# hallgeirl/cse168-raytracer

Measured on AMD Instinct MI355X. Metric: Mrays/s (primary+shadow), higher is better.
Workload: dtype f32; 1 GPU; sponza-standin 1920x1080 64spp primary+shadow; scene_triangles=76552, bvh_nodes=46701, math=exact: every quotient of the reference's slab and triangle tests, bit for bit, control_flow=while-while, ray_order=image order, resident_bytes_per_gpu=35765164

## Files before the change

cse168-raytracer_amd/csrc/mr_frame.hip:

```cpp
#include <hip/hip_runtime.h>

#include <cstring>

#include "mr_eye.h"
#include "mr_internal.h"
#include "mr_launch.h"
#include "mr_phong.h"
#include "mr_recursion.h"
#include "mr_surface.h"
#include "mr_tile.h"
#include "mr_traverse.h"

namespace mr {
namespace {

struct FrameArgs {
    EyeFrame eye;
    TraceParams tp;
    SurfacePtrs m;
    DirectLight lt;
    const float *mats;
    const uint32_t *prim_mat;
    mr_hit *hits;
    mr_hit *shadow_hits;
// ... 6 lines not shown
    uint32_t build, n_inner, n_rec;
};

__device__ __forceinline__ void eye_tables(const FrameArgs &a) {
    const unsigned i = blockIdx.x * (unsigned)kTraceBlock + threadIdx.x;
    const float ex = a.eye.eye[0], ey = a.eye.eye[1], ez = a.eye.eye[2];
    if (i < a.n_inner) {
        const float4 *q = a.tp.nodes + 4 * (size_t)i;
        const float4 q0 = q[0], q1 = q[1], q2 = q[2];
        int4 q3 = *reinterpret_cast<const int4 *>(q + 3);
        if (!(regular_pos(ex) && regular_pos(ey) && regular_pos(ez))) q3.z |= 1;
        float4 *d = a.rel_nodes + 4 * (size_t)i;
        d[0] = make_float4(q0.x - ex, q0.y - ex, q0.z - ey, q0.w - ey);
        d[1] = make_float4(q1.x - ex, q1.y - ex, q1.z - ey, q1.w - ey);
        d[2] = make_float4(q2.x - ez, q2.y - ez, q2.z - ez, q2.w - ez);
        *reinterpret_cast<int4 *>(d + 3) = q3;
    }
    if (i < a.n_rec) {
        const float4 *q = a.tp.tris + 3 * (size_t)i;
        const float4 q0 = q[0], q1 = q[1], q2 = q[2];
        const TriOriginTerms o = tri_origin_terms(q0, q1, q2, ex, ey, ez);
        float4 *d = a.rel_tris + 3 * (size_t)i;
        d[0] = make_float4(q2.y, q2.z, q2.w, o.pn);
        d[1] = make_float4(o.u.x, o.u.y, o.u.z, o.w.x);
        d[2] = make_float4(o.w.y, o.w.z, 0.0f, 0.0f);
    }
}

__device__ __forceinline__ unsigned tail_first_run(unsigned body_iters) {
    const unsigned q = body_iters >> 2;
    return q >= 8u ? 8u : q >= 4u ? 4u : q >= 2u ? 2u : 1u;
}
template <typename T>
__device__ __forceinline__ T kernarg_now(size_t offset) {
    typedef const volatile T __attribute__((address_space(4))) *ptr_t;
    const char __attribute__((address_space(4))) *ka = (const char __attribute__((address_space(4))) *)__builtin_amdgcn_kernarg_segment_ptr();
    return *(ptr_t)(ka + offset);
}

#ifndef MIRO_TAIL_PERMILLE
#define MIRO_TAIL_PERMILLE 60
#endif
#ifndef MIRO_BODY_ITERS
#define MIRO_BODY_ITERS 32
#endif
#ifndef MIRO_TAIL_MIN_CHUNKS
#define MIRO_TAIL_MIN_CHUNKS 60000ull
#endif
constexpr uint32_t kTailWgs = 1792 * (256 / kTraceBlock);
#ifndef MIRO_BODY_MIN_WGS
#define MIRO_BODY_MIN_WGS 14000
#endif
#ifndef MIRO_TAIL_PERMILLE_MID
#define MIRO_TAIL_PERMILLE_MID 60
#define MIRO_BODY_MIN_WGS_MID 14000
#endif
constexpr uint32_t kBodyMinWgs = MIRO_BODY_MIN_WGS;
struct FrameShape { uint32_t body_wgs, body_iters, tail_chunks, grid; };
inline FrameShape frame_schedule(unsigned long long chunks) {
    FrameShape s;
    if (chunks < MIRO_TAIL_MIN_CHUNKS || MIRO_TAIL_PERMILLE == 0 || kTraceBlock != 256) {
        const unsigned long long cap = chunks < kFrameLargeChunks ? (unsigned long long)kTraceGridCap : (unsigned long long)kFrameGridCapLarge;
        s.body_wgs = (uint32_t)(chunks < cap ? chunks : cap);
        s.body_iters = (uint32_t)((chunks + s.body_wgs - 1) / s.body_wgs);
        s.tail_chunks = 0;
        s.grid = s.body_wgs;
        return s;
    }
    const bool mid = chunks < kFrameLargeChunks;
    const unsigned long long tail_target = chunks * (mid ? MIRO_TAIL_PERMILLE_MID : MIRO_TAIL_PERMILLE) / 1000;
    uint32_t m = MIRO_BODY_ITERS;
    while (m > 1 && (chunks - tail_target) / m < (mid ? (uint32_t)MIRO_BODY_MIN_WGS_MID : kBodyMinWgs)) m >>= 1;
    while ((unsigned long long)m * (unsigned long long)kFrameGridCapLarge < chunks) m <<= 1;
    s.body_iters = m;
    s.body_wgs = (uint32_t)((chunks - tail_target) / m);
    s.tail_chunks = (uint32_t)(chunks - (unsigned long long)s.body_wgs * m);
    s.grid = s.body_wgs + kTailWgs;
    return s;
}

#if defined(MIRO_WG_TIMES) && MIRO_TRACE_BLOCK == 256
__device__ unsigned long long g_wg_times[4 * 131072];
#endif
template <int VAR, int SHADOW, bool MAT>
#ifndef MIRO_FRAME_WAVES
#define MIRO_FRAME_WAVES 7
#endif
__global__ __launch_bounds__(kTraceBlock) __attribute__((amdgpu_waves_per_eu(MIRO_FRAME_WAVES, 8))) void frame_kernel(FrameArgs a) {
#if defined(MIRO_WG_TIMES) && MIRO_TRACE_BLOCK == 256
    const unsigned long long wg_t0 = wall_clock64();
#endif
    constexpr bool kEyeRel = VAR == kTraceEyeRel;
    if (kEyeRel && a.build) {
        eye_tables(a);
        return;
    }
    extern __shared__ int s_stack[];
    __shared__ unsigned s_shadow_rays[kTraceBlock / 64];
    const int tid = threadIdx.x;
    const unsigned long long n = a.eye.n, n_round = (n + 63ull) & ~63ull;
    constexpr bool kObj = (VAR & kVarObjects) != 0;
    const uint32_t spp = a.eye.spp;
    const float inv_spp = 1.0f / (float)spp;
    Stats st = {0ull, 0ull};
    unsigned my_shadow_rays = 0;

    __shared__ unsigned s_pull, s_run[2];
    if (tid == 0) { s_run[0] = 0; s_run[1] = 0; }
    unsigned long long idx, stride, limit;
    if (blockIdx.x < a.body_wgs) {
        const unsigned long long body_end = (unsigned long long)a.body_wgs * a.body_iters * kTraceBlock;
        idx = (unsigned long long)xcd_block_id_of(blockIdx.x, a.body_wgs, a.body_wgs >= (unsigned)kFrameGridCapLarge || a.tail_chunks != 0, a.tail_chunks != 0 ? 4096u : kXcdMinGrid) * kTraceBlock + tid;
        stride = (unsigned long long)a.body_wgs * kTraceBlock;
        limit = body_end < n_round ? body_end : n_round;
    } else {
        idx = 0; stride = 0; limit = n_round;
    }
    for (;; idx += stride) {
        if (__builtin_expect(stride == 0, 0)) {
            if (tid == 0) {
                unsigned left = s_run[1], next = s_run[0] + 1u;
                if (left == 0) {
                    const unsigned T = kernarg_now<uint32_t>(offsetof(FrameArgs, tail_chunks));
                    unsigned k = atomicAdd(kernarg_now<unsigned *>(offsetof(FrameArgs, tail_counter)), 1u);
                    s_pull = k;
                    unsigned at = 0;
                    next = 0xFFFFFFFFu;
                    for (unsigned size = tail_first_run(kernarg_now<uint32_t>(offsetof(FrameArgs, body_iters))); size >= 1; size >>= 1) {
                        const unsigned runs = size > 1 ? T / (4u * size) : T - at;
                        if (k < runs) { next = at + k * size; left = size; break; }
                        k -= runs;
                        at += runs * size;
                    }
                }
                s_run[0] = next;
                s_run[1] = next == 0xFFFFFFFFu ? 0u : left - 1u;
            }
            __syncthreads();
            const unsigned c = s_run[0];
            __syncthreads();
            if (c == 0xFFFFFFFFu) break;
            idx = ((unsigned long long)kernarg_now<uint32_t>(offsetof(FrameArgs, tail_base)) + c) * kTraceBlock + tid;
            if (idx >= limit) continue;
        } else if (idx >= limit) break;
        const bool live = idx < n;
        uint32_t x = 0, row = 0, y = 0, sm = 0;
        float4 ra = make_float4(0.f, 0.f, 0.f, 0.f), rb = make_float4(1.f, 1.f, 1.f, -1.f);
        if (live) {
            eye_sample_of(a.eye, idx, x, row, y, sm);
            eye_ray_of(a.eye, x, y, sm, ra, rb);
        }
        mr_hit h;
        {
            RayRegs r;
            ray_setup(r, ra, rb);
            Lane L;
            int plane_hit;
            if (kEyeRel) {
                TraceParams tp = a.tp;
                tp.nodes = a.rel_nodes; tp.tris = a.rel_tris;
                for (int k = 0; k < 3; k++) {
                    tp.root_lo[k] = kernarg_now<float>(offsetof(FrameArgs, rel_root_lo) + 4 * k);
                    tp.root_hi[k] = kernarg_now<float>(offsetof(FrameArgs, rel_root_hi) + 4 * k);
                }
                trace_ray<true, false, false, VAR, kEyeRel>(tp, r, rb.w, live, L, plane_hit, s_stack, tid, st);
            } else {
                trace_ray<true, false, false, VAR>(a.tp, r, rb.w, live, L, plane_hit, s_stack, tid, st);
            }
            h = make_hit<kObj>(a.tp, L, plane_hit, rb.w);
        }
        if (a.hits && live) reinterpret_cast<float4 *>(a.hits)[idx] = *reinterpret_cast<const float4 *>(&h);

        const bool hit = live && h.prim != MR_MISS;
        float c[3] = {0.f, 0.f, 0.f}, highlight = 0.0f;
        if (live && !hit) { c[0] = a.lt.bg[0]; c[1] = a.lt.bg[1]; c[2] = a.lt.bg[2]; }
        float4 sa = make_float4(0.f, 0.f, 0.f, 0.f), sb = make_float4(1.f, 1.f, 1.f, -1.f);
        if (hit) {
            float P[3], N[3];
            const float ox = kEyeRel ? a.eye.eye[0] : ra.x, oy = kEyeRel ? a.eye.eye[1] : ra.y, oz = kEyeRel ? a.eye.eye[2] : ra.z;
            if (MAT) {
                rec::MeshMat mm;
                mm.s = a.m; mm.mats = a.mats; mm.prim_mat = a.prim_mat;
                LightArgs la;
                for (int k = 0; k < 3; k++) { la.L[k] = a.lt.L[k]; la.color[k] = a.lt.color[k]; }
                la.wattage = a.lt.wattage;
                rec::surface_point_od(mm, ox, oy, oz, rb.x, rb.y, rb.z, h.t, h.prim, h.beta, h.gamma, P, N);
                phong_terms(la, rec::material_of(mm, h.prim), P, N, rb.x, rb.y, rb.z, c, highlight);
            } else {
                surface_od<true>(a.m, ox, oy, oz, rb.x, rb.y, rb.z, h.t, h.prim, h.beta, h.gamma, P, N);
            }
            if (SHADOW != 2) shadow_ray_of(P, a.lt.L[0], a.lt.L[1], a.lt.L[2], sa, sb);
            if (!MAT) phong_direct(a.lt, P, N, rb.x, rb.y, rb.z, c);
            if (SHADOW != 2) my_shadow_rays++;
        }
        if (SHADOW != 2) {
            RayRegs r;
            ray_setup(r, sa, sb);
            Lane L;
            int plane_hit;
            trace_ray<true, SHADOW == 1, false, VAR>(a.tp, r, sb.w, hit, L, plane_hit, s_stack, tid, st);
            mr_hit hs = make_hit<kObj>(a.tp, L, plane_hit, sb.w);
            if (!hit) { hs.t = 0.0f; hs.prim = MR_MISS; hs.beta = 0.0f; hs.gamma = 0.0f; }
            if (a.shadow_hits && live) reinterpret_cast<float4 *>(a.shadow_hits)[idx] = *reinterpret_cast<const float4 *>(&hs);
            if (MAT) {
                if (hit) {
                    rec::MeshMat mm;
                    mm.s = a.m; mm.mats = a.mats; mm.prim_mat = a.prim_mat;
                    phong_combine(c, highlight, light_scale_of(mm, sa, sb, *reinterpret_cast<const float4 *>(&hs)), c);
                }
            } else if (hs.prim != MR_MISS) {
                c[0] = 0.f; c[1] = 0.f; c[2] = 0.f;
            }
        } else {
            if (a.shadow_hits && live) reinterpret_cast<float4 *>(a.shadow_hits)[idx] = make_float4(0.0f, __uint_as_float(MR_MISS), 0.0f, 0.0f);
            if (MAT && hit) phong_combine(c, highlight, 1.0f, c);
        }
        for (uint32_t off = 1; off < spp; off <<= 1) {
            c[0] += __shfl_xor(c[0], (int)off, 64);
            c[1] += __shfl_xor(c[1], (int)off, 64);
            c[2] += __shfl_xor(c[2], (int)off, 64);
        }
        if (live) eye_sample_of(a.eye, idx, x, row, y, sm);
        if (live && sm == 0) {
            if (spp > 1) { c[0] *= inv_spp; c[1] *= inv_spp; c[2] *= inv_spp; }
            float *o = a.rgb + 3 * ((size_t)row * a.eye.W + x);
            o[0] = c[0]; o[1] = c[1]; o[2] = c[2];
        }
    }

    if (stride == 0 && tid == 0) {
        const unsigned readers = gridDim.x - kernarg_now<uint32_t>(offsetof(FrameArgs, body_wgs));
        const unsigned T = kernarg_now<uint32_t>(offsetof(FrameArgs, tail_chunks));
        unsigned runs = 0, at = 0;
        for (unsigned size = tail_first_run(kernarg_now<uint32_t>(offsetof(FrameArgs, body_iters))); size >= 1; size >>= 1) {
            const unsigned r = size > 1 ? T / (4u * size) : T - at;
            runs += r;
            at += r * size;
        }
        if (s_pull == runs + readers - 1u) atomicExch(kernarg_now<unsigned *>(offsetof(FrameArgs, tail_counter)), 0u);
    }
    if (a.counts) {
        unsigned w = my_shadow_rays;
        for (int off = 32; off > 0; off >>= 1) w += __shfl_down(w, off, 64);
        if ((tid & 63) == 0) s_shadow_rays[tid >> 6] = w;
        __syncthreads();
        if (tid == 0) {
            unsigned long long tot = 0;
            for (int k = 0; k < kTraceBlock / 64; k++) tot += s_shadow_rays[k];
            if (tot) atomicAdd(&a.counts[1], tot);
            if (blockIdx.x == 0) atomicAdd(&a.counts[0], n);
        }
    }
#if defined(MIRO_WG_TIMES) && MIRO_TRACE_BLOCK == 256
    if (tid == 0 && blockIdx.x < 131072u) {
        g_wg_times[4 * blockIdx.x] = wg_t0;
        g_wg_times[4 * blockIdx.x + 1] = wall_clock64();
        g_wg_times[4 * blockIdx.x + 2] = __builtin_amdgcn_s_getreg((31 << 11) | 4);
        g_wg_times[4 * blockIdx.x + 3] = __builtin_amdgcn_s_getreg((31 << 11) | 20);
    }
#endif
}
#if defined(MIRO_WG_TIMES) && MIRO_TRACE_BLOCK == 256
}
}
extern "C" int mr_debug_wg_times(unsigned long long *out, unsigned n_words) {
    return (int)hipMemcpyFromSymbol(out, HIP_SYMBOL(mr::g_wg_times), (size_t)n_words * 8, 0, hipMemcpyDeviceToHost);
}
namespace mr {
namespace {
#endif

template <int VAR, int SHADOW, bool MAT>
mr_status launch_frame_t(FrameArgs a, hipStream_t stream) {
    size_t lds = 0;
    const mr_status st = stack_lds(&frame_kernel<VAR, SHADOW, MAT>, a.tp.stack_depth, kStackLdsShared, lds);
    if (st != MR_OK) return st;
    const FrameShape shape = frame_schedule((a.eye.n + kTraceBlock - 1) / kTraceBlock);
    a.body_wgs = shape.body_wgs; a.body_iters = shape.body_iters; a.tail_chunks = shape.tail_chunks;
    a.tail_base = shape.body_wgs * shape.body_iters;
    if (shape.tail_chunks && !a.tail_counter) return fail(MR_ERR_STATE, "mr_render_direct: no hand-out counter for the tail of a large frame");
    hipLaunchKernelGGL((frame_kernel<VAR, SHADOW, MAT>), dim3(shape.grid), dim3(kTraceBlock), lds, stream, a);
    MR_HIP_CHECK(hipGetLastError());
    return MR_OK;
}

template <int VAR>
mr_status launch_frame_plain(const FrameArgs &a, bool any, hipStream_t stream) {
    return any ? launch_frame_t<VAR, 1, false>(a, stream) : launch_frame_t<VAR, 0, false>(a, stream);
}
template <int VAR>
mr_status launch_frame_default(const FrameArgs &a, bool any, bool no_shadows, bool mat, hipStream_t stream) {
    if (mat) return no_shadows ? launch_frame_t<VAR, 2, true>(a, stream) : launch_frame_t<VAR, 0, true>(a, stream);
    if (no_shadows) return launch_frame_t<VAR, 2, false>(a, stream);
    return launch_frame_plain<VAR>(a, any, stream);
}

}

#ifndef MR_FRAME_ENTRY
#define MR_FRAME_ENTRY launch_frame_b256
#endif
static mr_status eye_tables_for(const DeviceScene &ds, EyeTablePool &pool, FrameArgs &a, hipStream_t stream) {
    hipStreamCaptureStatus cs = hipStreamCaptureStatusNone;
    MR_HIP_CHECK(hipStreamIsCapturing(stream, &cs));
    const bool capturing = cs != hipStreamCaptureStatusNone;
    std::lock_guard<std::mutex> lock(pool.mu);
    const uint64_t call = ++pool.calls;
    EyeTables *e = nullptr;
    if (!capturing)
        for (EyeTables &c : pool.set)
            if (c.reusable && memcmp(c.eye, a.eye.eye, sizeof(c.eye)) == 0) { e = &c; break; }
    const bool build = e == nullptr;
    if (build) {
        e = &pool.set[0];
        for (EyeTables &c : pool.set)
            if (c.last_use < e->last_use) e = &c;
        e->reusable = false;
        if (!e->d || !e->ready) {
            hipStreamCaptureMode mode = hipStreamCaptureModeRelaxed;
            MR_HIP_CHECK(hipThreadExchangeStreamCaptureMode(&mode));
            hipError_t err = e->d ? hipSuccess : hipMalloc(reinterpret_cast<void **>(&e->d), eye_table_bytes(ds));
            if (err == hipSuccess && !e->ready)
                err = hipEventCreateWithFlags(reinterpret_cast<hipEvent_t *>(&e->ready), hipEventDisableTiming);
            MR_HIP_CHECK(hipThreadExchangeStreamCaptureMode(&mode));
            MR_HIP_CHECK(err);
        }
    } else if (e->stream != (void *)stream) {
        MR_HIP_CHECK(hipStreamWaitEvent(stream, static_cast<hipEvent_t>(e->ready), 0));
    }
    e->last_use = call;
    a.rel_nodes = e->d;
    a.rel_tris = e->d + 4 * (size_t)ds.n_inner;
    for (int c = 0; c < 3; c++) { a.rel_root_lo[c] = ds.root_lo[c] - a.eye.eye[c]; a.rel_root_hi[c] = ds.root_hi[c] - a.eye.eye[c]; }
    if (!build) return MR_OK;
    FrameArgs b = a;
    b.build = 1; b.n_inner = ds.n_inner; b.n_rec = ds.n_tris;
    const uint32_t n = ds.n_inner > ds.n_tris ? ds.n_inner : ds.n_tris;
    if (n) {
        hipLaunchKernelGGL((frame_kernel<kTraceEyeRel, 0, false>), dim3((n + kTraceBlock - 1) / kTraceBlock), dim3(kTraceBlock), 0, stream, b);
        MR_HIP_CHECK(hipGetLastError());
    }
    if (capturing) e->captured = true;
    if (!e->captured) {
        MR_HIP_CHECK(hipEventRecord(static_cast<hipEvent_t>(e->ready), stream));
// ... 68 lines not shown
```

cse168-raytracer_amd/csrc/mr_traverse.h:

```cpp
#pragma once

#include <hip/hip_runtime.h>

#include "mr_internal.h"
#include "mr_launch.h"

namespace mr {
namespace {

#ifndef MIRO_CAP_LARGE
#define MIRO_CAP_LARGE 65536
#define MIRO_RUN_LARGE 256
#endif
constexpr int kFrameGridCapLarge = MIRO_CAP_LARGE;
constexpr unsigned long long kFrameLargeChunks = 1ull << 18;

#ifndef MIRO_XCD_MIN_GRID
#define MIRO_XCD_MIN_GRID 16384
#endif
constexpr unsigned kXcdRun = 64, kXcdRunLarge = MIRO_RUN_LARGE, kXcdMinGrid = MIRO_XCD_MIN_GRID;
__device__ __forceinline__ unsigned xcd_block_id_of(unsigned b, unsigned G, bool large, unsigned min_grid = kXcdMinGrid) {
    if (G < min_grid) return b;
    const unsigned run = large ? kXcdRunLarge : kXcdRun;
    const unsigned xcd = b & 7u, slot = b >> 3, grp = slot / run, k = slot - grp * run;
    return (grp + 1u) * (8u * run) <= G ? grp * (8u * run) + xcd * run + k : b;
}
__device__ __forceinline__ unsigned xcd_block_id() {
    return xcd_block_id_of(blockIdx.x, gridDim.x, gridDim.x >= (unsigned)kFrameGridCapLarge);
}
constexpr float kEps = 1e-4f;
constexpr float kInf = __builtin_huge_valf();

struct Stats { unsigned long long box, tri; };

template <bool STRICT>
__device__ __forceinline__ void slab_axis(float lo, float hi, float o, float d, float inv, float &mn, float &mx) {
    float t0, t1;
    if (STRICT) { t0 = (lo - o) / d; t1 = (hi - o) / d; }
    else        { t0 = (lo - o) * inv; t1 = (hi - o) * inv; }
    const bool m = t0 > t1;
    const float tnear = m ? t1 : t0, tfar = m ? t0 : t1;
    if (tnear > mn) mn = tnear;
    if (tfar < mx) mx = tfar;
}

struct RayRegs {
    float ox, oy, oz, dx, dy, dz;
    float ix, iy, iz;
    float mx_, my_, mz_;
    float tmin;
    float nox, noy, noz;
};

__device__ __forceinline__ void ray_setup(RayRegs &r, const float4 ra, const float4 rb) {
    r.ox = ra.x; r.oy = ra.y; r.oz = ra.z; r.tmin = ra.w;
    r.dx = rb.x; r.dy = rb.y; r.dz = rb.z;
    r.ix = 1.0f / r.dx; r.iy = 1.0f / r.dy; r.iz = 1.0f / r.dz;
    r.mx_ = -r.dx; r.my_ = -r.dy; r.mz_ = -r.dz;
    r.nox = -(r.ox * r.ix); r.noy = -(r.oy * r.iy); r.noz = -(r.oz * r.iz);
}

__device__ __forceinline__ bool lane_is_nan_free(const RayRegs &r) {
    return (__builtin_fabsf(r.ox) < kInf) && (__builtin_fabsf(r.oy) < kInf) && (__builtin_fabsf(r.oz) < kInf) &&
           (__builtin_fabsf(r.dx) < kInf) && (__builtin_fabsf(r.dy) < kInf) && (__builtin_fabsf(r.dz) < kInf) &&
           (__builtin_fabsf(r.ix) < kInf) && (__builtin_fabsf(r.iy) < kInf) && (__builtin_fabsf(r.iz) < kInf) &&
           (__builtin_fabsf(r.nox) < kInf) && (__builtin_fabsf(r.noy) < kInf) && (__builtin_fabsf(r.noz) < kInf);
}

__device__ __forceinline__ float vmax3(float a, float b, float c) {
    float o;
    asm("v_max3_f32 %0, %1, %2, %3" : "=v"(o) : "v"(a), "v"(b), "v"(c));
    return o;
}
__device__ __forceinline__ float vmin3(float a, float b, float c) {
    float o;
    asm("v_min3_f32 %0, %1, %2, %3" : "=v"(o) : "v"(a), "v"(b), "v"(c));
    return o;
}

__device__ __forceinline__ float vmax2(float a, float b) {
    float o;
    asm("v_max_f32 %0, %1, %2" : "=v"(o) : "v"(a), "v"(b));
    return o;
}
__device__ __forceinline__ float vmin2(float a, float b) {
    float o;
    asm("v_min_f32 %0, %1, %2" : "=v"(o) : "v"(a), "v"(b));
    return o;
}

__device__ __forceinline__ unsigned vsad(float a, float b) {
    unsigned o;
    asm("v_sad_u32 %0, %1, %2, 0" : "=v"(o) : "v"(a), "v"(b));
    return o;
}
__device__ __forceinline__ unsigned vmin3u(unsigned a, unsigned b, unsigned c) {
    unsigned o;
    asm("v_min3_u32 %0, %1, %2, %3" : "=v"(o) : "v"(a), "v"(b), "v"(c));
    return o;
}

__device__ __forceinline__ void slab_box_minmax(float lox, float hix, float loy, float hiy, float loz, float hiz,
                                                const RayRegs &r, float &mn, float &mx) {
    const float ax = (lox - r.ox) * r.ix, bx = (hix - r.ox) * r.ix;
    const float ay = (loy - r.oy) * r.iy, by = (hiy - r.oy) * r.iy;
    const float az = (loz - r.oz) * r.iz, bz = (hiz - r.oz) * r.iz;
    mn = vmax3(vmin2(ax, bx), vmin2(ay, by), vmin2(az, bz));
    mx = vmin3(vmax2(ax, bx), vmax2(ay, by), vmax2(az, bz));
}

__device__ __forceinline__ float exact_quot(float a, float d, float inv) {
    const float q = a * inv;
    return __builtin_fmaf(__builtin_fmaf(-q, d, a), inv, q);
}

__device__ __forceinline__ void slab_box_exactq(float lox, float hix, float loy, float hiy, float loz, float hiz,
// ... 116 lines not shown
    const float t0 = (-b - sq) / (2.0f * a), t1 = (-b + sq) / (2.0f * a);
    if ((t0 > r.tmin) && (t0 < tmax)) { t = t0; return true; }
    if ((t1 > r.tmin) && (t1 < tmax)) { t = t1; return true; }
    return false;
}

template <bool EXACT, bool OBJ, bool REL = false>
__device__ __forceinline__ bool object_test(const float4 q0, const float4 q1, const float4 q2, const RayRegs &r,
                                            float tmax, float &t, float &beta, float &gamma) {
    static_assert(!REL || (EXACT && !OBJ), "eye-relative records hold exact triangle tests only");
    if (REL) return tri_test_rel(q0, q1, make_float2(q2.x, q2.y), r, tmax, t, beta, gamma);
    if (OBJ && __float_as_uint(q2.w) == kSphereTag) {
        beta = 0.0f; gamma = 0.0f;
        return sphere_test(q0, r, tmax, t);
    }
    return tri_test<EXACT>(q0, q1, q2, r, tmax, t, beta, gamma);
}

constexpr int kDone = (int)0x80000000;
constexpr int kStackStride = kTraceBlock * (int)sizeof(int);
struct Lane {
    float best_t, best_b, best_g;
    int best_pos;
    int sp, cur;
    int lpos, lend;
    __device__ __forceinline__ bool have() const { return cur != kDone; }
};

typedef __attribute__((address_space(3))) int lds_int;
__device__ __forceinline__ void stack_push(Lane &L, int *s_stack, int v) {
    *reinterpret_cast<lds_int *>((unsigned)L.sp) = v;
    L.sp += kStackStride;
}
__device__ __forceinline__ int stack_pop(Lane &L, int *s_stack) {
    L.sp -= kStackStride;
    return *reinterpret_cast<lds_int *>((unsigned)L.sp);
}
__device__ __forceinline__ void stack_reset(Lane &L, int *s_stack, int tid) {
    L.sp = (int)(unsigned)reinterpret_cast<__UINTPTR_TYPE__>((lds_int *)s_stack) + tid * (int)sizeof(int);
    stack_push(L, s_stack, kDone);
}

typedef float v16f __attribute__((ext_vector_type(16)));
__device__ __forceinline__ v16f load_node_scalar(const float4 *nodes, int cur_uniform) {
    const float4 *ptr = nodes + 4 * (size_t)cur_uniform;
    v16f v;
    asm volatile("s_load_dwordx16 %0, %1, 0x0\n\ts_waitcnt lgkmcnt(0)" : "=s"(v) : "s"(ptr) : "memory");
    return v;
}

template <bool EXACT, bool STATS, int SLAB, int OCT = 8>
__device__ __forceinline__ void node_slabs(const float4 q0, const float4 q1, const float4 q2, const RayRegs &r,
                                           float &mn0, float &mx0, float &mn1, float &mx1);
template <bool EXACT, bool STATS, int SLAB, int OCT = 8>
__device__ __forceinline__ void node_slabs_guarded(const float4 q0, const float4 q1, const float4 q2, const RayRegs &r, float best_t,
                                                   float &mn0, float &mx0, float &mn1, float &mx1, float &k0, float &k1);

template <bool STATS, bool SAFE, bool HAVE_K = false>
__device__ __forceinline__ void node_decide(float mn0, float mx0, float mn1, float mx1, int ref0, int ref1,
                                            const RayRegs &r, Lane &L, int *s_stack, Stats &st, float k0 = 0.0f, float k1 = 0.0f) {
    bool h0, h1;
    if (SAFE) {
        if (!HAVE_K) { k0 = vmin2(mx0, L.best_t); k1 = vmin2(mx1, L.best_t); }
        h0 = !((mn0 > k0) || (mx0 < r.tmin));
        h1 = !((mn1 > k1) || (mx1 < r.tmin));
    } else {
        h0 = !((mn0 > mx0) || (mn0 > L.best_t) || (mx0 < r.tmin));
        h1 = !((mn1 > mx1) || (mn1 > L.best_t) || (mx1 < r.tmin));
    }
    const bool one_first = h1 && (!h0 || (mn0 > mn1));
    if (h0 && h1) {
        stack_push(L, s_stack, one_first ? ref0 : ref1);
        L.cur = one_first ? ref1 : ref0;
        if (STATS) st.box++;
    } else if (h0 || h1) {
        L.cur = h0 ? ref0 : ref1;
        if (STATS) st.box++;
    } else {
        L.cur = stack_pop(L, s_stack);
        if (STATS && L.cur != kDone) st.box++;
    }
}

template <bool EXACT, bool STATS, int SLAB, bool SCALAR = false, int OCT = 8>
__device__ __forceinline__ void node_step(const TraceParams &p, const RayRegs &r, Lane &L, int *s_stack, int tid, Stats &st) {
    float mn0, mx0, mn1, mx1;
    constexpr bool kSafe = SLAB == 1 || SLAB == 2 || SLAB == 4 || SLAB == 5 || SLAB == 6;
    constexpr bool kGuarded = SLAB == 5 || SLAB == 6;
    if (SCALAR) {
        const int cur0 = __builtin_amdgcn_readfirstlane(L.cur);
        if (__all(L.cur == cur0)) {
            const v16f v = load_node_scalar(p.nodes, cur0);
            const float4 q0 = make_float4(v[0], v[1], v[2], v[3]), q1 = make_float4(v[4], v[5], v[6], v[7]);
            const float4 q2 = make_float4(v[8], v[9], v[10], v[11]);
            if ((SLAB == 4 || kGuarded) && __float_as_int(v[14]) != 0) {
                node_slabs<EXACT, STATS, 3>(q0, q1, q2, r, mn0, mx0, mn1, mx1);
                node_decide<STATS, false>(mn0, mx0, mn1, mx1, __float_as_int(v[12]), __float_as_int(v[13]), r, L, s_stack, st);
                return;
            }
            float k0 = 0.0f, k1 = 0.0f;
            node_slabs_guarded<EXACT, STATS, SLAB, OCT>(q0, q1, q2, r, L.best_t, mn0, mx0, mn1, mx1, k0, k1);
            node_decide<STATS, kSafe, kGuarded>(mn0, mx0, mn1, mx1, __float_as_int(v[12]), __float_as_int(v[13]), r, L, s_stack, st, k0, k1);
            return;
        }
    }
    const float4 *nd = p.nodes + 4 * (size_t)L.cur;
    const float4 q0 = nd[0], q1 = nd[1], q2 = nd[2];
    const int4 q3 = *reinterpret_cast<const int4 *>(nd + 3);
    if ((SLAB == 4 || kGuarded) && q3.z != 0) {
        node_slabs<EXACT, STATS, 3>(q0, q1, q2, r, mn0, mx0, mn1, mx1);
        node_decide<STATS, false>(mn0, mx0, mn1, mx1, q3.x, q3.y, r, L, s_stack, st);
        return;
    }
    float k0 = 0.0f, k1 = 0.0f;
    node_slabs_guarded<EXACT, STATS, SLAB, OCT>(q0, q1, q2, r, L.best_t, mn0, mx0, mn1, mx1, k0, k1);
    node_decide<STATS, kSafe, kGuarded>(mn0, mx0, mn1, mx1, q3.x, q3.y, r, L, s_stack, st, k0, k1);
}

template <bool EXACT, bool STATS, int SLAB, int OCT>
__device__ __forceinline__ void node_slabs(const float4 q0, const float4 q1, const float4 q2, const RayRegs &r,
                                           float &mn0, float &mx0, float &mn1, float &mx1) {
    if (OCT < 8 && (SLAB == 1 || SLAB == 2 || SLAB == 4)) {
        slab_box_oct<OCT, SLAB>(q0.x, q0.y, q0.z, q0.w, q2.x, q2.y, r, mn0, mx0);
        slab_box_oct<OCT, SLAB>(q1.x, q1.y, q1.z, q1.w, q2.z, q2.w, r, mn1, mx1);
    } else if (SLAB == 2) {
        slab_box_lean(q0.x, q0.y, q0.z, q0.w, q2.x, q2.y, r, mn0, mx0);
        slab_box_lean(q1.x, q1.y, q1.z, q1.w, q2.z, q2.w, r, mn1, mx1);
    } else if (SLAB == 4) {
        slab_box_exactq(q0.x, q0.y, q0.z, q0.w, q2.x, q2.y, r, mn0, mx0);
        slab_box_exactq(q1.x, q1.y, q1.z, q1.w, q2.z, q2.w, r, mn1, mx1);
    } else if (EXACT && (SLAB == 0 || SLAB == 3)) {
        mn0 = -kInf; mx0 = kInf; mn1 = -kInf; mx1 = kInf;
        slab_axis<SLAB == 3>(q0.x, q0.y, r.ox, r.dx, r.ix, mn0, mx0);
        slab_axis<SLAB == 3>(q0.z, q0.w, r.oy, r.dy, r.iy, mn0, mx0);
        slab_axis<SLAB == 3>(q2.x, q2.y, r.oz, r.dz, r.iz, mn0, mx0);
        slab_axis<SLAB == 3>(q1.x, q1.y, r.ox, r.dx, r.ix, mn1, mx1);
        slab_axis<SLAB == 3>(q1.z, q1.w, r.oy, r.dy, r.iy, mn1, mx1);
        slab_axis<SLAB == 3>(q2.z, q2.w, r.oz, r.dz, r.iz, mn1, mx1);
    } else {
        slab_box_minmax(q0.x, q0.y, q0.z, q0.w, q2.x, q2.y, r, mn0, mx0);
        slab_box_minmax(q1.x, q1.y, q1.z, q1.w, q2.z, q2.w, r, mn1, mx1);
    }
}

template <bool EXACT, bool STATS, int SLAB, int OCT>
__device__ __forceinline__ void node_slabs_guarded(const float4 q0, const float4 q1, const float4 q2, const RayRegs &r, float best_t,
                                                   float &mn0, float &mx0, float &mn1, float &mx1, float &k0, float &k1) {
    if (SLAB != 5 && SLAB != 6) {
        node_slabs<EXACT, STATS, SLAB, OCT>(q0, q1, q2, r, mn0, mx0, mn1, mx1);
        return;
    }
    node_slabs<EXACT, STATS, 1, OCT>(q0, q1, q2, r, mn0, mx0, mn1, mx1);
    unsigned near, t0, t1;
    if (SLAB == 6) {
        asm("v_min_f32 %3, %7, %9\n\tv_min_f32 %4, %8, %9\n\t"
            "v_sad_u32 %0, %5, %3, 0\n\tv_sad_u32 %1, %6, %4, 0\n\tv_sad_u32 %2, %5, %6, 0\n\tv_min3_u32 %0, %0, %1, %2"
            : "=&v"(near), "=&v"(t0), "=&v"(t1), "=&v"(k0), "=&v"(k1)
            : "v"(mn0), "v"(mn1), "v"(mx0), "v"(mx1), "v"(best_t));
    } else {
        asm("v_min_f32 %3, %8, %10\n\tv_min_f32 %4, %9, %10\n\t"
            "v_sad_u32 %0, %5, %3, 0\n\tv_sad_u32 %1, %8, %6, 0\n\tv_sad_u32 %2, %7, %4, 0\n\tv_min3_u32 %0, %0, %1, %2\n\t"
            "v_sad_u32 %1, %9, %6, 0\n\tv_sad_u32 %2, %5, %7, 0\n\tv_min3_u32 %0, %0, %1, %2"
            : "=&v"(near), "=&v"(t0), "=&v"(t1), "=&v"(k0), "=&v"(k1)
            : "v"(mn0), "v"(r.tmin), "v"(mn1), "v"(mx0), "v"(mx1), "v"(best_t));
    }
    if (__any(near <= 16u)) {
        node_slabs<EXACT, STATS, 4, OCT>(q0, q1, q2, r, mn0, mx0, mn1, mx1);
        k0 = vmin2(mx0, best_t); k1 = vmin2(mx1, best_t);
    }
}

typedef float v4f __attribute__((ext_vector_type(4)));
__device__ __forceinline__ void load_tri_scalar(const float4 *tris, unsigned pos_uniform, float4 &q0, float4 &q1, float4 &q2) {
    const float4 *ptr = tris + 3 * (size_t)pos_uniform;
    v4f a, b, c;
    asm volatile("s_load_dwordx4 %0, %3, 0x0\n\ts_load_dwordx4 %1, %3, 0x10\n\ts_load_dwordx4 %2, %3, 0x20\n\ts_waitcnt lgkmcnt(0)"
                 : "=&s"(a), "=&s"(b), "=&s"(c) : "s"(ptr) : "memory");
    q0 = make_float4(a[0], a[1], a[2], a[3]);
    q1 = make_float4(b[0], b[1], b[2], b[3]);
    q2 = make_float4(c[0], c[1], c[2], c[3]);
}
typedef float v2f __attribute__((ext_vector_type(2)));
__device__ __forceinline__ void load_tri_rel_scalar(const float4 *tris, unsigned pos_uniform, float4 &q0, float4 &q1, float4 &q2) {
    const float4 *ptr = tris + 3 * (size_t)pos_uniform;
    v4f a, b;
    v2f c;
    asm volatile("s_load_dwordx4 %0, %3, 0x0\n\ts_load_dwordx4 %1, %3, 0x10\n\ts_load_dwordx2 %2, %3, 0x20\n\ts_waitcnt lgkmcnt(0)"
                 : "=&s"(a), "=&s"(b), "=&s"(c) : "s"(ptr) : "memory");
// ... 50 lines not shown
            if (ok && t < L.best_t) {
                L.best_t = t; L.best_b = b; L.best_g = g; L.best_pos = (int)(first + k);
                if (ANY) { done = true; break; }
            }
        }
    }
    if (STATS) {
        if (OBJ) {
            for (unsigned k = 0; k < cnt; k++)
                if (__float_as_uint(p.tris[3 * (size_t)(first + k) + 2].w) != kSphereTag) st.tri++;
        } else {
            st.tri += cnt;
        }
    }
    if (ANY && done) {
        L.cur = kDone;
    } else {
        L.cur = stack_pop(L, s_stack);
        if (STATS && L.cur != kDone) st.box++;
    }
}

template <bool EXACT, bool ANY, bool STATS, bool SCALAR, bool OBJ, bool REL = false>
__device__ __forceinline__ void tri_step(const TraceParams &p, const RayRegs &r, Lane &L, int *s_stack, Stats &st) {
    bool done = false;
    if (SCALAR) {
        const int cur0 = __builtin_amdgcn_readfirstlane(L.cur);
        if (__all(L.cur == cur0 && L.lpos == L.lend)) {
            const unsigned bits0 = ~(unsigned)cur0;
            const unsigned first0 = bits0 >> kLeafCountBits;
            unsigned cnt0 = bits0 & kLeafCountMask;
            if (cnt0 == kLeafCountMask) cnt0 = p.leaf_cnt_ext[first0];
            for (unsigned k = 0; k < cnt0; k++) {
                float4 q0, q1, q2;
                load_tri_uniform<REL>(p.tris, first0 + k, q0, q1, q2);
                if (!(ANY && done)) {
                    float t, b, g;
                    const bool ok = object_test<EXACT, OBJ, REL>(q0, q1, q2, r, L.best_t, t, b, g);
                    if (ok && t < L.best_t) {
                        L.best_t = t; L.best_b = b; L.best_g = g; L.best_pos = (int)(first0 + k);
                        if (ANY) done = true;
                    }
                }
            }
            if (STATS) {
                if (OBJ) { for (unsigned k = 0; k < cnt0; k++) if (__float_as_uint(p.tris[3 * (size_t)(first0 + k) + 2].w) != kSphereTag) st.tri++; }
                else st.tri += cnt0;
            }
            if (ANY && done) { L.cur = kDone; }
            else { L.cur = stack_pop(L, s_stack); if (STATS && L.cur != kDone) st.box++; }
            return;
        }
    }
    if (L.lpos == L.lend) {
        const unsigned bits = ~(unsigned)L.cur;
        const unsigned first = bits >> kLeafCountBits;
        unsigned cnt = bits & kLeafCountMask;
        if (cnt == kLeafCountMask) cnt = p.leaf_cnt_ext[first];
        L.lpos = (int)first; L.lend = (int)(first + cnt);
        if (STATS) {
            if (OBJ) { for (unsigned k = 0; k < cnt; k++) if (__float_as_uint(p.tris[3 * (size_t)(first + k) + 2].w) != kSphereTag) st.tri++; }
            else st.tri += cnt;
        }
    }
    if (L.lpos < L.lend) {
        float4 q0, q1, q2;
        load_tri<REL>(p.tris + 3 * (size_t)L.lpos, q0, q1, q2);
        float t, b, g;
        const bool ok = object_test<EXACT, OBJ, REL>(q0, q1, q2, r, L.best_t, t, b, g);
        if (ok && t < L.best_t) {
            L.best_t = t; L.best_b = b; L.best_g = g; L.best_pos = L.lpos;
            if (ANY) done = true;
        }
        L.lpos++;
    }
    if (ANY && done) {
        L.cur = kDone; L.lpos = L.lend;
    } else if (L.lpos == L.lend) {
        L.cur = stack_pop(L, s_stack);
        if (STATS && L.cur != kDone) st.box++;
    }
}

template <bool EXACT, bool ANY, bool STATS, int SLAB, int MODE, bool SCALAR, bool OBJ = false, int OCT = 8, bool REL = false>
__device__ __forceinline__ void traverse(const TraceParams &p, const RayRegs &r, Lane &L, int *s_stack, int tid, Stats &st) {
    if (MODE == 2) {
        L.lpos = 0; L.lend = 0;
        while (true) {
            const bool want_node = L.cur >= 0, want_tri = L.cur < 0 && L.cur != kDone;
            const unsigned long long m_node = __ballot(want_node), m_tri = __ballot(want_tri);
            if ((m_node | m_tri) == 0ull) break;
            if (__popcll(m_node) >= __popcll(m_tri)) {
                if (want_node) node_step<EXACT, STATS, SLAB, SCALAR, OCT>(p, r, L, s_stack, tid, st);
            } else {
                if (want_tri) tri_step<EXACT, ANY, STATS, SCALAR, OBJ, REL>(p, r, L, s_stack, st);
            }
        }
    } else if (MODE == 1) {
        while (__any(L.have())) {
            while (L.cur >= 0) node_step<EXACT, STATS, SLAB, SCALAR, OCT>(p, r, L, s_stack, tid, st);
            if (L.have()) leaf_step<EXACT, ANY, STATS, SCALAR, OBJ, REL>(p, r, L, s_stack, tid, st);
        }
    } else {
        while (L.have()) {
            if (L.cur >= 0) node_step<EXACT, STATS, SLAB, SCALAR>(p, r, L, s_stack, tid, st);
            else leaf_step<EXACT, ANY, STATS, false, OBJ, REL>(p, r, L, s_stack, tid, st);
        }
    }
}

template <bool EXACT, bool ANY, bool STATS, int VAR, bool REL = false>
__device__ __forceinline__ void trace_ray(const TraceParams &p, const RayRegs &r_in, float tmax0, bool live, Lane &L,
                                          int &plane_hit, int *s_stack, int tid, Stats &st) {
    static_assert(!REL || ((VAR & kVarStrict) && !(VAR & kVarObjects) && !STATS), "eye-relative tables: default traversal, triangles only");
    RayRegs r = r_in;
    if (REL) { r.ox = 0.0f; r.oy = 0.0f; r.oz = 0.0f; }
    constexpr bool kStrict = STATS || (VAR & kVarStrict);
    constexpr int kBaseSlab = kStrict ? 3 : 0;
    constexpr bool kMinMax = !kStrict && (VAR & kVarMinMax);
    constexpr int kWW = (VAR & kVarVote) ? 2 : ((VAR & kVarWhileWhile) ? 1 : 0);
    constexpr int kSafeSlab = (VAR & kVarLeanFma) ? 2 : 1;
    constexpr bool kScalar = (VAR & kVarScalar) != 0;
    constexpr bool kObj = (VAR & kVarObjects) != 0;

    L.best_t = tmax0;
    L.best_b = 0.0f; L.best_g = 0.0f;
    L.best_pos = -1;
    stack_reset(L, s_stack, tid);
    {
        float mn = -kInf, mx = kInf;
        slab_axis<kStrict>(p.root_lo[0], p.root_hi[0], r.ox, r.dx, r.ix, mn, mx);
        slab_axis<kStrict>(p.root_lo[1], p.root_hi[1], r.oy, r.dy, r.iy, mn, mx);
        slab_axis<kStrict>(p.root_lo[2], p.root_hi[2], r.oz, r.dz, r.iz, mn, mx);
        if (STATS && live) st.box++;
        L.cur = (live && !((mn > mx) || (mn > tmax0) || (mx < r.tmin))) ? p.root_ref : kDone;
    }

    constexpr bool kOct = (VAR & kVarOctant) != 0;
    constexpr int kExactSlab = (VAR & kVarGuarded) ? 5 : 4;
    constexpr int kGoodSlab = kMinMax ? kSafeSlab : kExactSlab;
    constexpr int kOctSlab = kGoodSlab == 5 ? 6 : kGoodSlab;
    const bool good_wave = kMinMax ? __all(lane_is_nan_free(r) || !live) : ((kStrict && !STATS) ? __all(lane_is_regular(r) || !live) : false);
    bool done_oct = false;
    if (kOct && (kMinMax || (kStrict && !STATS)) && good_wave) {
        const unsigned long long m_live = __ballot(live);
        if (m_live) {
            const int oct = octant_of(r);
            const int oct0 = __builtin_amdgcn_readlane(oct, __ffsll((long long)m_live) - 1);
            if (__all(!live || oct == oct0) && (kOctSlab != 6 || __all(!live || r.tmin == 0.0f))) {
                done_oct = true;
                switch (oct0) {
                    case 0: traverse<EXACT, ANY, STATS, kOctSlab, kWW, kScalar, kObj, 0, REL>(p, r, L, s_stack, tid, st); break;
                    case 1: traverse<EXACT, ANY, STATS, kOctSlab, kWW, kScalar, kObj, 1, REL>(p, r, L, s_stack, tid, st); break;
                    case 2: traverse<EXACT, ANY, STATS, kOctSlab, kWW, kScalar, kObj, 2, REL>(p, r, L, s_stack, tid, st); break;
                    case 3: traverse<EXACT, ANY, STATS, kOctSlab, kWW, kScalar, kObj, 3, REL>(p, r, L, s_stack, tid, st); break;
                    case 4: traverse<EXACT, ANY, STATS, kOctSlab, kWW, kScalar, kObj, 4, REL>(p, r, L, s_stack, tid, st); break;
                    case 5: traverse<EXACT, ANY, STATS, kOctSlab, kWW, kScalar, kObj, 5, REL>(p, r, L, s_stack, tid, st); break;
                    case 6: traverse<EXACT, ANY, STATS, kOctSlab, kWW, kScalar, kObj, 6, REL>(p, r, L, s_stack, tid, st); break;
                    default: traverse<EXACT, ANY, STATS, kOctSlab, kWW, kScalar, kObj, 7, REL>(p, r, L, s_stack, tid, st); break;
                }
            }
        }
    }
    if (done_oct) {
    } else if (kMinMax) {
        if (good_wave) traverse<EXACT, ANY, STATS, kSafeSlab, kWW, kScalar, kObj>(p, r, L, s_stack, tid, st);
        else traverse<EXACT, ANY, STATS, 0, kWW, false, kObj>(p, r, L, s_stack, tid, st);
    } else if (kStrict && !STATS) {
        constexpr int kMixedFlow = ((VAR & kVarMixedVote) && kWW == 1) ? 2 : kWW;
        if (good_wave) traverse<EXACT, ANY, STATS, 4, kMixedFlow, kScalar, kObj, 8, REL>(p, r, L, s_stack, tid, st);
        else traverse<EXACT, ANY, STATS, 3, kWW, kScalar, kObj, 8, REL>(p, r, L, s_stack, tid, st);
    } else {
        traverse<EXACT, ANY, STATS, kBaseSlab, kWW, kStrict && kScalar, kObj>(p, r, L, s_stack, tid, st);
    }

    plane_hit = -1;
    if (kObj && live && !(ANY && L.best_pos >= 0)) {
        for (uint32_t k = 0; k < p.n_planes; k++) {
            const float4 pn = p.planes[2 * k], po = p.planes[2 * k + 1];
            const float ndotd = (pn.x * r.dx + pn.y * r.dy) + pn.z * r.dz;
            if ((double)__builtin_fabsf(ndotd) < 1e-6) continue;
            const float t = ((pn.x * (po.x - r.ox) + pn.y * (po.y - r.oy)) + pn.z * (po.z - r.oz)) / ndotd;
            if (t < r.tmin || t > tmax0) continue;
            if ((L.best_pos < 0 && plane_hit < 0) || t < L.best_t) { L.best_t = t; plane_hit = (int)k; }
        }
    }
}

template <bool OBJ>
__device__ __forceinline__ mr_hit make_hit(const TraceParams &p, const Lane &L, int plane_hit, float tmax0) {
    mr_hit h;
    if (OBJ && plane_hit >= 0) {
        h.t = L.best_t; h.prim = kPlaneBit | (uint32_t)plane_hit; h.beta = 0.0f; h.gamma = 0.0f;
    } else if (L.best_pos >= 0) {
        h.t = L.best_t; h.prim = p.tri_prim[L.best_pos]; h.beta = L.best_b; h.gamma = L.best_g;
    } else {
        h.t = tmax0; h.prim = MR_MISS; h.beta = 0.0f; h.gamma = 0.0f;
    }
    return h;
}

template <bool EXACT, bool ANY, bool STATS, int VAR, bool REL = false>
__device__ __forceinline__ mr_hit trace_hit(const TraceParams &p, const float4 &ra, const float4 &rb, float tmax, bool live,
                                            int *s_stack, int tid, Stats &st) {
    RayRegs r;
    ray_setup(r, ra, rb);
    Lane L;
    int plane_hit;
    trace_ray<EXACT, ANY, STATS, VAR, REL>(p, r, tmax, live, L, plane_hit, s_stack, tid, st);
    return make_hit<(VAR & kVarObjects) != 0>(p, L, plane_hit, tmax);
}

__device__ __forceinline__ unsigned long long whole_workgroups(unsigned long long n) {
    return (n + (unsigned long long)kTraceBlock - 1ull) / kTraceBlock * kTraceBlock;
}

template <int BLOCK, int WORDS>
__device__ __forceinline__ void workgroup_add(const unsigned (&mine)[WORDS], unsigned long long *counters) {
    __shared__ unsigned s_part[WORDS][BLOCK / 64];
    const int tid = threadIdx.x;
    unsigned w[WORDS];
    for (int j = 0; j < WORDS; j++) w[j] = mine[j];
    for (int off = 32; off > 0; off >>= 1)
        for (int j = 0; j < WORDS; j++) w[j] += __shfl_down(w[j], off, 64);
    if ((tid & 63) == 0)
        for (int j = 0; j < WORDS; j++) s_part[j][tid >> 6] = w[j];
    __syncthreads();
    if (tid < WORDS) {
        unsigned long long tot = 0;
        for (int k = 0; k < BLOCK / 64; k++) tot += s_part[tid][k];
        if (tot) atomicAdd(&counters[tid], tot);
    }
}
template <int BLOCK>
__device__ __forceinline__ void workgroup_add(unsigned mine, unsigned long long *counter) {
    const unsigned m[1] = {mine};
    workgroup_add<BLOCK, 1>(m, counter);
}

}
}
```

Before: 17890 Mrays/s.

## Add wave-uniform BVH descent loop for coherent octant traversal

```diff
diff --git a/cse168-raytracer_amd/csrc/mr_frame.hip b/cse168-raytracer_amd/csrc/mr_frame.hip
--- a/cse168-raytracer_amd/csrc/mr_frame.hip
+++ b/cse168-raytracer_amd/csrc/mr_frame.hip
@@ -112,6 +112,9 @@
 #if defined(MIRO_WG_TIMES) && MIRO_TRACE_BLOCK == 256
 __device__ unsigned long long g_wg_times[4 * 131072];
 #endif
+#if defined(MIRO_RUN_COUNTS)
+__device__ unsigned long long g_run_counts[3];
+#endif
 template <int VAR, int SHADOW, bool MAT>
 #ifndef MIRO_FRAME_WAVES
 #define MIRO_FRAME_WAVES 7
@@ -121,6 +124,7 @@
     const unsigned long long wg_t0 = wall_clock64();
 #endif
     constexpr bool kEyeRel = VAR == kTraceEyeRel;
+    constexpr bool kRun = kEyeRel && !MAT;
     if (kEyeRel && a.build) {
         eye_tables(a);
         return;
@@ -193,7 +197,7 @@
                     tp.root_lo[k] = kernarg_now<float>(offsetof(FrameArgs, rel_root_lo) + 4 * k);
                     tp.root_hi[k] = kernarg_now<float>(offsetof(FrameArgs, rel_root_hi) + 4 * k);
                 }
-                trace_ray<true, false, false, VAR, kEyeRel>(tp, r, rb.w, live, L, plane_hit, s_stack, tid, st);
+                trace_ray<true, false, false, VAR, kEyeRel, kRun>(tp, r, rb.w, live, L, plane_hit, s_stack, tid, st);
             } else {
                 trace_ray<true, false, false, VAR>(a.tp, r, rb.w, live, L, plane_hit, s_stack, tid, st);
             }
@@ -228,7 +232,7 @@
             ray_setup(r, sa, sb);
             Lane L;
             int plane_hit;
-            trace_ray<true, SHADOW == 1, false, VAR>(a.tp, r, sb.w, hit, L, plane_hit, s_stack, tid, st);
+            trace_ray<true, SHADOW == 1, false, VAR, false, kRun>(a.tp, r, sb.w, hit, L, plane_hit, s_stack, tid, st);
             mr_hit hs = make_hit<kObj>(a.tp, L, plane_hit, sb.w);
             if (!hit) { hs.t = 0.0f; hs.prim = MR_MISS; hs.beta = 0.0f; hs.gamma = 0.0f; }
             if (a.shadow_hits && live) reinterpret_cast<float4 *>(a.shadow_hits)[idx] = *reinterpret_cast<const float4 *>(&hs);
@@ -281,6 +285,12 @@
             if (blockIdx.x == 0) atomicAdd(&a.counts[0], n);
         }
     }
+#if defined(MIRO_RUN_COUNTS)
+    {
+        const unsigned mine[3] = {st.node_steps, st.run_visits, st.run_splits};
+        workgroup_add<kTraceBlock, 3>(mine, g_run_counts);
+    }
+#endif
 #if defined(MIRO_WG_TIMES) && MIRO_TRACE_BLOCK == 256
     if (tid == 0 && blockIdx.x < 131072u) {
         g_wg_times[4 * blockIdx.x] = wg_t0;
@@ -290,6 +300,22 @@
     }
 #endif
 }
+#if defined(MIRO_RUN_COUNTS)
+}
+}
+#if MIRO_TRACE_BLOCK == 256
+#define MR_RUN_COUNTS_ENTRY mr_debug_run_counts_b256
+#else
+#define MR_RUN_COUNTS_ENTRY mr_debug_run_counts_b128
+#endif
+extern "C" int MR_RUN_COUNTS_ENTRY(unsigned long long *out) {
+    const unsigned long long zero[3] = {0ull, 0ull, 0ull};
+    const int e = (int)hipMemcpyFromSymbol(out, HIP_SYMBOL(mr::g_run_counts), sizeof(zero), 0, hipMemcpyDeviceToHost);
+    return e ? e : (int)hipMemcpyToSymbol(HIP_SYMBOL(mr::g_run_counts), zero, sizeof(zero), 0, hipMemcpyHostToDevice);
+}
+namespace mr {
+namespace {
+#endif
 #if defined(MIRO_WG_TIMES) && MIRO_TRACE_BLOCK == 256
 }
 }
diff --git a/cse168-raytracer_amd/csrc/mr_traverse.h b/cse168-raytracer_amd/csrc/mr_traverse.h
--- a/cse168-raytracer_amd/csrc/mr_traverse.h
+++ b/cse168-raytracer_amd/csrc/mr_traverse.h
@@ -31,7 +31,17 @@
 constexpr float kEps = 1e-4f;
 constexpr float kInf = __builtin_huge_valf();
 
+#ifdef MIRO_RUN_COUNTS
+struct Stats { unsigned long long box, tri; unsigned node_steps, run_visits, run_splits; };
+__device__ __forceinline__ void run_count_once(unsigned &c) {
+    const int lane = (int)__lane_id();
+    if (__builtin_amdgcn_readfirstlane(lane) == lane) c++;
+}
+#define MR_RUN_COUNT(field) run_count_once(field)
+#else
 struct Stats { unsigned long long box, tri; };
+#define MR_RUN_COUNT(field) ((void)0)
+#endif
 
 template <bool STRICT>
 __device__ __forceinline__ void slab_axis(float lo, float hi, float o, float d, float inv, float &mn, float &mx) {
@@ -314,7 +324,53 @@
     }
 }
 
-template <bool EXACT, bool STATS, int SLAB, bool SCALAR = false, int OCT = 8>
+template <bool EXACT, int OCT>
+__device__ __forceinline__ void uniform_run(const TraceParams &p, const RayRegs &r, Lane &L, int *s_stack, Stats &st, int cur) {
+    const unsigned long long m_all = __builtin_amdgcn_ballot_w64(true);
+    float mn0, mx0, mn1, mx1, k0, k1;
+    int node, ref0, ref1;
+    bool regular;
+    do {
+        node = cur;
+        const v16f v = load_node_scalar(p.nodes, node);
+        const float4 q0 = make_float4(v[0], v[1], v[2], v[3]), q1 = make_float4(v[4], v[5], v[6], v[7]);
+        const float4 q2 = make_float4(v[8], v[9], v[10], v[11]);
+        ref0 = __float_as_int(v[12]); ref1 = __float_as_int(v[13]);
+        regular = __float_as_int(v[14]) == 0;
+        MR_RUN_COUNT(st.run_visits);
+        cur = kDone;
+        if (regular) {
+            k0 = 0.0f; k1 = 0.0f;
+            node_slabs_guarded<EXACT, false, 6, OCT>(q0, q1, q2, r, L.best_t, mn0, mx0, mn1, mx1, k0, k1);
+            const unsigned long long out0 = (__builtin_amdgcn_ballot_w64(mn0 > k0) | __builtin_amdgcn_ballot_w64(mx0 < r.tmin)) & m_all;
+            const unsigned long long out1 = (__builtin_amdgcn_ballot_w64(mn1 > k1) | __builtin_amdgcn_ballot_w64(mx1 < r.tmin)) & m_all;
+            if ((out0 | out1) == 0ull) {
+                const unsigned long long one_first = __builtin_amdgcn_ballot_w64(mn0 > mn1);
+                if (one_first == 0ull) { stack_push(L, s_stack, ref1); cur = ref0; }
+                else if (one_first == m_all) { stack_push(L, s_stack, ref0); cur = ref1; }
+            } else if ((out0 | (out1 ^ m_all)) == 0ull) {
+                cur = ref0;
+            } else if ((out1 | (out0 ^ m_all)) == 0ull) {
+                cur = ref1;
+            }
+        }
+    } while (cur >= 0);
+    if (cur != kDone) {
+        L.cur = cur;
+    } else if (!regular) {
+        const v16f v = load_node_scalar(p.nodes, node);
+        const float4 q0 = make_float4(v[0], v[1], v[2], v[3]), q1 = make_float4(v[4], v[5], v[6], v[7]);
+        const float4 q2 = make_float4(v[8], v[9], v[10], v[11]);
+        node_slabs<EXACT, false, 3>(q0, q1, q2, r, mn0, mx0, mn1, mx1);
+        node_decide<false, false>(mn0, mx0, mn1, mx1, ref0, ref1, r, L, s_stack, st);
+    } else {
+        if (((unsigned long long)__builtin_amdgcn_ballot_w64((mn0 > k0) || (mx0 < r.tmin)) &
+             (unsigned long long)__builtin_amdgcn_ballot_w64((mn1 > k1) || (mx1 < r.tmin))) != m_all) MR_RUN_COUNT(st.run_splits);
+        node_decide<false, true, true>(mn0, mx0, mn1, mx1, ref0, ref1, r, L, s_stack, st, k0, k1);
+    }
+}
+
+template <bool EXACT, bool STATS, int SLAB, bool SCALAR = false, int OCT = 8, bool RUN = false>
 __device__ __forceinline__ void node_step(const TraceParams &p, const RayRegs &r, Lane &L, int *s_stack, int tid, Stats &st) {
     float mn0, mx0, mn1, mx1;
     constexpr bool kSafe = SLAB == 1 || SLAB == 2 || SLAB == 4 || SLAB == 5 || SLAB == 6;
@@ -322,6 +378,11 @@
     if (SCALAR) {
         const int cur0 = __builtin_amdgcn_readfirstlane(L.cur);
         if (__all(L.cur == cur0)) {
+            if (RUN && SLAB == 6 && OCT < 8 && !STATS) {
+                uniform_run<EXACT, OCT>(p, r, L, s_stack, st, cur0);
+                return;
+            }
+            MR_RUN_COUNT(st.node_steps);
             const v16f v = load_node_scalar(p.nodes, cur0);
             const float4 q0 = make_float4(v[0], v[1], v[2], v[3]), q1 = make_float4(v[4], v[5], v[6], v[7]);
             const float4 q2 = make_float4(v[8], v[9], v[10], v[11]);
@@ -336,6 +397,7 @@
             return;
         }
     }
+    MR_RUN_COUNT(st.node_steps);
     const float4 *nd = p.nodes + 4 * (size_t)L.cur;
     const float4 q0 = nd[0], q1 = nd[1], q2 = nd[2];
     const int4 q3 = *reinterpret_cast<const int4 *>(nd + 3);
@@ -552,7 +614,7 @@
     }
 }
 
-template <bool EXACT, bool ANY, bool STATS, int SLAB, int MODE, bool SCALAR, bool OBJ = false, int OCT = 8, bool REL = false>
+template <bool EXACT, bool ANY, bool STATS, int SLAB, int MODE, bool SCALAR, bool OBJ = false, int OCT = 8, bool REL = false, bool RUN = false>
 __device__ __forceinline__ void traverse(const TraceParams &p, const RayRegs &r, Lane &L, int *s_stack, int tid, Stats &st) {
     if (MODE == 2) {
         L.lpos = 0; L.lend = 0;
@@ -568,7 +630,7 @@
         }
     } else if (MODE == 1) {
         while (__any(L.have())) {
-            while (L.cur >= 0) node_step<EXACT, STATS, SLAB, SCALAR, OCT>(p, r, L, s_stack, tid, st);
+            while (L.cur >= 0) node_step<EXACT, STATS, SLAB, SCALAR, OCT, RUN>(p, r, L, s_stack, tid, st);
             if (L.have()) leaf_step<EXACT, ANY, STATS, SCALAR, OBJ, REL>(p, r, L, s_stack, tid, st);
         }
     } else {
@@ -579,7 +641,7 @@
     }
 }
 
-template <bool EXACT, bool ANY, bool STATS, int VAR, bool REL = false>
+template <bool EXACT, bool ANY, bool STATS, int VAR, bool REL = false, bool RUN = false>
 __device__ __forceinline__ void trace_ray(const TraceParams &p, const RayRegs &r_in, float tmax0, bool live, Lane &L,
                                           int &plane_hit, int *s_stack, int tid, Stats &st) {
     static_assert(!REL || ((VAR & kVarStrict) && !(VAR & kVarObjects) && !STATS), "eye-relative tables: default traversal, triangles only");
@@ -620,14 +682,14 @@
             if (__all(!live || oct == oct0) && (kOctSlab != 6 || __all(!live || r.tmin == 0.0f))) {
                 done_oct = true;
                 switch (oct0) {
-                    case 0: traverse<EXACT, ANY, STATS, kOctSlab, kWW, kScalar, kObj, 0, REL>(p, r, L, s_stack, tid, st); break;
-                    case 1: traverse<EXACT, ANY, STATS, kOctSlab, kWW, kScalar, kObj, 1, REL>(p, r, L, s_stack, tid, st); break;
-                    case 2: traverse<EXACT, ANY, STATS, kOctSlab, kWW, kScalar, kObj, 2, REL>(p, r, L, s_stack, tid, st); break;
-                    case 3: traverse<EXACT, ANY, STATS, kOctSlab, kWW, kScalar, kObj, 3, REL>(p, r, L, s_stack, tid, st); break;
-                    case 4: traverse<EXACT, ANY, STATS, kOctSlab, kWW, kScalar, kObj, 4, REL>(p, r, L, s_stack, tid, st); break;
-                    case 5: traverse<EXACT, ANY, STATS, kOctSlab, kWW, kScalar, kObj, 5, REL>(p, r, L, s_stack, tid, st); break;
-                    case 6: traverse<EXACT, ANY, STATS, kOctSlab, kWW, kScalar, kObj, 6, REL>(p, r, L, s_stack, tid, st); break;
-                    default: traverse<EXACT, ANY, STATS, kOctSlab, kWW, kScalar, kObj, 7, REL>(p, r, L, s_stack, tid, st); break;
+                    case 0: traverse<EXACT, ANY, STATS, kOctSlab, kWW, kScalar, kObj, 0, REL, RUN>(p, r, L, s_stack, tid, st); break;
+                    case 1: traverse<EXACT, ANY, STATS, kOctSlab, kWW, kScalar, kObj, 1, REL, RUN>(p, r, L, s_stack, tid, st); break;
+                    case 2: traverse<EXACT, ANY, STATS, kOctSlab, kWW, kScalar, kObj, 2, REL, RUN>(p, r, L, s_stack, tid, st); break;
+                    case 3: traverse<EXACT, ANY, STATS, kOctSlab, kWW, kScalar, kObj, 3, REL, RUN>(p, r, L, s_stack, tid, st); break;
+                    case 4: traverse<EXACT, ANY, STATS, kOctSlab, kWW, kScalar, kObj, 4, REL, RUN>(p, r, L, s_stack, tid, st); break;
+                    case 5: traverse<EXACT, ANY, STATS, kOctSlab, kWW, kScalar, kObj, 5, REL, RUN>(p, r, L, s_stack, tid, st); break;
+                    case 6: traverse<EXACT, ANY, STATS, kOctSlab, kWW, kScalar, kObj, 6, REL, RUN>(p, r, L, s_stack, tid, st); break;
+                    default: traverse<EXACT, ANY, STATS, kOctSlab, kWW, kScalar, kObj, 7, REL, RUN>(p, r, L, s_stack, tid, st); break;
                 }
             }
         }
```

Measured after the change: 19120 Mrays/s (median of 6 runs). 6.9% higher.
